# flanglet/kanzi

Measured on AMD Instinct MI355X. Metric: encode+decode MB/s, 4 MiB-block synthetic stream, BWT+RANK+ZRLT & ANS0 (level-5 core chain), bit-exact .knz, higher is better.
Workload: dtype u8; 1 GPU; configs[2]: BWT+RANK+ZRLT & ANS0, 2048 x 4194304 B blocks per GPU per step (64 distinct synthetic blocks per GPU, SURVEY 8d generator standing in for silesia.tar, tiled), blocks round-robin over ranks; block_size=4194304, parallelism=blocks%1, round_trip_ok=True

## Files before the change

kanzi_amd/csrc/kz_api.hip:

```cpp
#include <dirent.h>
#include "kz_pipe.h"
#include <stdlib.h>
#include <thread>
#include <sched.h>

extern "C" int32_t kz_abi_version(void) { return KZ_ABI_VERSION; }

extern "C" kz_ctx* kz_ctx_create(int32_t deviceId) {
  int ndev = 0;
  if (hipGetDeviceCount(&ndev) != hipSuccess || ndev <= 0) return nullptr;
  if (deviceId < 0 || deviceId >= ndev) return nullptr;
  if (hipSetDevice(deviceId) != hipSuccess) return nullptr;
  kz_ctx* ctx = new kz_ctx();
  ctx->device = deviceId;
  { int cus = 0; if (hipDeviceGetAttribute(&cus, hipDeviceAttributeMultiprocessorCount, deviceId) == hipSuccess && cus > 0) ctx->numCUs = cus; }
  if (hipStreamCreateWithFlags(&ctx->stream, hipStreamNonBlocking) != hipSuccess) { delete ctx; return nullptr; }
  if (hipHostMalloc((void**)&ctx->hpin, 1 << 20, hipHostMallocDefault) != hipSuccess) { hipStreamDestroy(ctx->stream); delete ctx; return nullptr; }
  ctx->hpinInts = (1 << 20) / 4;
  kz_switches_read(ctx->sw);
  {
    const int hw = (int)std::thread::hardware_concurrency();
    ctx->blockingWaits = ctx->sw.blockingWaits >= 0 ? ctx->sw.blockingWaits : ((hw > 0 && kz_usable_cpus() < hw) ? 1 : 0);
  }
  return ctx;
}
void kz_switches_read(kz_switches& s) {
  s = kz_switches();
  auto num = [](const char* name, int unset) { const char* e = getenv(name); return e ? atoi(e) : unset; };
  auto flag = [](const char* name) { return getenv(name) != nullptr ? 1 : 0; };
  auto digit = [](const char* name, int lo, int hi, int unset) { const char* e = getenv(name); return (e && e[0] >= '0' + lo && e[0] <= '0' + hi) ? e[0] - '0' : unset; };
  { const char* e = getenv("KZ_BLOCKING_WAITS"); s.blockingWaits = e ? (atoi(e) ? 1 : 0) : -1; }
  s.textGpu = digit("KZ_TEXT_GPU", 0, 3, -1);
  s.textGpuMin = num("KZ_TEXT_GPU_MIN", 512);
  s.textFwdGpu = digit("KZ_TEXT_FWD_GPU", 0, 1, -1);
  s.textFwdGpuMin = num("KZ_TEXT_FWD_GPU_MIN", 256);
  s.text1FwdGpu = digit("KZ_TEXT1_FWD_GPU", 0, 1, -1);
  s.text1FwdGpuMin = num("KZ_TEXT1_FWD_GPU_MIN", 64);
  s.utfGpu = digit("KZ_UTF_GPU", 0, 0, 1);
  s.utfFwdGpu = digit("KZ_UTF_FWD_GPU", 0, 1, -1);
  s.textGpuTrace = flag("KZ_TEXT_GPU_TRACE");
  s.fuseMinBlocks = num("KZ_FUSE_MIN_BLOCKS", 32);
  s.overlapClasses = num("KZ_OVERLAP_CLASSES", 3);
  { const char* e = getenv("KZ_WIDE_QUEUES"); s.wideQueues = e ? (atoi(e) ? 1 : 0) : -1; }
  s.noSFirst = flag("KZ_NO_SFIRST");
  s.traceSched = flag("KZ_TRACE_SCHED");
  s.tracePipe = flag("KZ_TRACE_PIPE");
  s.hostChunk = num("KZ_HOST_CHUNK", 0);
  { const int v = num("KZ_HOST_CHUNK_DEC", 512); s.hostChunkDec = v < 8 ? 8 : v; }
  { const char* e = getenv("KZ_HOST_INV_STAGED"); s.hostInvStaged = e ? atoi(e) : -1; }
  s.streamChunk = num("KZ_STREAM_CHUNK", 0);
  s.streamSerial = flag("KZ_STREAM_SERIAL");
  s.readScatter = flag("KZ_READ_SCATTER");
  s.writeGather = flag("KZ_WRITE_GATHER");
  s.bwtTrie = num("KZ_BWT_TRIE", -1); s.bwtTrieWin = num("KZ_BWT_TRIEWIN", -1); s.bwtBuckets = num("KZ_BWT_BUCKETS", -1);
  s.bwtDmax = num("KZ_BWT_DMAX", -1); s.bwtRetire = num("KZ_BWT_RETIRE", -1); s.bwtLazyRank = num("KZ_BWT_LAZYRANK", -1);
  s.bwtTrace = flag("KZ_BWT_TRACE");
  s.bwtTestTrieOverflow = digit("KZ_BWT_TEST_TRIE_OVERFLOW", 0, 9, -1);
  s.cmTestRowBytes = num("KZ_CM_TEST_ROW_BYTES", 0);
  { const char* f = getenv("KZ_FPAQ_FORCE"); s.fpaqForce = f ? ((f[0] == 'w' || f[0] == 'W' || f[0] == '1') ? 1 : ((f[0] == 'l' || f[0] == 'L' || f[0] == '2') ? 2 : 0)) : 0; }
  s.sbrtForm = num("KZ_SBRT_FORM", -1);
}
extern "C" void kz_ctx_reload_switches(kz_ctx* ctx) {
  if (!ctx) return;
  kz_switches_read(ctx->sw);
  if (ctx->sw.blockingWaits >= 0) ctx->blockingWaits = ctx->sw.blockingWaits;
}
extern "C" void kz_ctx_destroy(kz_ctx* ctx) {
  if (!ctx) return;
  if (ctx->worker.joinable()) {
    { std::lock_guard<std::mutex> g(ctx->qmu); ctx->stopWorker = true; }
    ctx->qcv.notify_all();
    ctx->worker.join();
  }
  hipSetDevice(ctx->device);
  if (ctx->arena) hipFree(ctx->arena);
  for (int i = 0; i < 5; i++) { if (ctx->side[i]) hipStreamDestroy(ctx->side[i]); if (ctx->evJoin[i]) hipEventDestroy(ctx->evJoin[i]); }
  if (ctx->hpin) hipHostFree(ctx->hpin);
  for (int i = 0; i < 2; i++) {
    if (ctx->pinIn[i].p) hipHostFree(ctx->pinIn[i].p);
    if (ctx->pinOut[i].p) hipHostFree(ctx->pinOut[i].p);
    if (ctx->hsIn[i].p) hipHostFree(ctx->hsIn[i].p);
    if (ctx->hsOut[i].p) hipHostFree(ctx->hsOut[i].p);
    if (ctx->tfOut[i].p) hipHostFree(ctx->tfOut[i].p);
    if (ctx->hiAux[i].p) hipFree(ctx->hiAux[i].p);
    if (ctx->hiStream[i]) hipStreamDestroy(ctx->hiStream[i]);
    if (ctx->devIn[i].p) hipFree(ctx->devIn[i].p);
    if (ctx->devOut[i].p) hipFree(ctx->devOut[i].p);
  }
// ... 357 lines not shown
```

kanzi_amd/csrc/kz_bwt_fwd.h:

```cpp
#pragma once
#include "kz_device.h"
#include "kz_internal.h"
#include <utility>

#define BW_LIVE 0x80000000u

typedef unsigned long long u64;
typedef uint32_t u32;
typedef uint8_t u8;
typedef u64 __attribute__((aligned(1))) bw_u64_unaligned;

struct BwtArrays {
  u64* key[2]; u32* val[2];
  u32* rank; u32* sa;
  u32* tileHist;
  u32* digitBase;
  u32* bucketCnt;
  int32_t* d_w;
  int32_t* d_big;
  u32* tileA;
  u32* tileB;
  u32* tileLive;
  int32_t* d_n;
  int32_t* d_m;
// ... 135 lines not shown
      const u32 r1 = run + c0;
      if (c1) gdelta[j + 1] = V.bStart[j + 1] + atomicAdd(&V.bFill[j + 1], c1) - r1;
      tc2[j >> 1] = run | (r1 << 16);
      run = r1 + c1;
    }
    if (threadIdx.x == 0) scan[31] = total;
  }
  __syncthreads();
  const u32 total = scan[31];
#pragma unroll
  for (int r = 0; r < TILE_ / 1024; r++) {
    if (bp[r] != 0xFFFFFFFFu) {
      const u32 bk = bp[r] & 0xFFFFu;
      const u32 w = tc2[bk >> 1];
      const u32 slot = ((bk & 1u) ? (w >> 16) : (w & 0xFFFFu)) + (bp[r] >> 16);
      stage[slot] = el[r]; stageB[slot] = (uint16_t)bk;
    }
  }
  __syncthreads();
#pragma unroll
  for (int r = 0; r < TILE_ / 1024; r++) {
    const u32 slot = (u32)r * 1024 + threadIdx.x;
    if (slot < total) elem[gdelta[stageB[slot]] + slot] = stage[slot];
  }
}

struct BwtRun {
  kz_ctx* ctx; kz_batch* bt;
  BwtArrays A; TrieArrays TR;
  int B, maxN, T; int64_t NS;
  int bitsR, bitsG, nBuckets, Dmax;
  bool useBuckets, useTrie;
  bool noRetire, trieWinOff, lazyRank, trace; int forceOvfRound;
  u64 *kC, *kF; u32 *vC, *vF;
  void swap() { std::swap(kC, kF); std::swap(vC, vF); }
  int nAct;
  int32_t *h_act, *d_act;
  int mMax, wMax;
  int h; bool windowed;
};
static inline int gridFor(int n, int per) { int g = (n + per - 1) / per; return g < 1 ? 1 : g; }

bool tr_applies(int maxN);
size_t bwt_trie_scratch(int maxN);
bool bwt_trie_alloc(kz_ctx* ctx, int B, int maxN, TrieArrays& TR);
int bwt_trie_text_round(BwtRun& R);
int bwt_trie_key_round(BwtRun& R);
```

kanzi_amd/csrc/kz_bwt_fwd.hip:

```cpp
#include "kz_bwt_fwd.h"
#include <stdlib.h>
#include <algorithm>

#define RS_ITEMS 16
#define RS_TILE (KZ_WG * RS_ITEMS)
#define RSORT_TILE 16384
#define RSORT_ITEMS (RSORT_TILE / KZ_WG)

__device__ __forceinline__ u64 bw_text_key(const u8* __restrict__ s, int i, int n, int K) {
  u64 k = __builtin_bswap64(*(const bw_u64_unaligned*)(s + i)) >> (8 * (8 - K));
  const int rem = n - i;
  if (rem < K) k &= ~0ULL << (8 * (K - rem));
  return k;
}
struct TextSrc { const u8* src; int64_t stride; int K; };
__global__ void k_bwt_init(BwtArrays A, int B) {
  const int b = blockIdx.x * blockDim.x + threadIdx.x;
  if (b < B) { A.d_m[b] = A.d_n[b]; A.d_w[b] = 0; }
}

#define MSD_BINS 1024
template <int BINS, bool MSD, bool TEXT>
__device__ __forceinline__ void radix_hist_body(const u64* __restrict__ keyIn, const BwtArrays& A, int shift, TextSrc X) {
  const int b = bw_row_block(A, blockIdx.y);
// ... 12 lines not shown
    const int idx = base + r * KZ_WG + threadIdx.x;
    const bool valid = idx < m;
    const u32 d = valid ? (u32)(((TEXT ? bw_text_key(X.src + (int64_t)b * X.stride, idx, m, X.K) : key[idx]) >> shift) & (BINS - 1)) : 0;
    const uint64_t vm = kz_ballot(valid);
    const u32 d0 = (u32)__builtin_amdgcn_readfirstlane((int)d);
    if (vm != 0 && kz_ballot(valid && d == d0) == vm) { if (lane == (int)__builtin_ctzll(vm)) atomicAdd(&hist[d0], (u32)__popcll(vm)); }
    else if (valid) atomicAdd(&hist[d], 1u);
  }
  __syncthreads();
  u32* th = A.tileHist + (int64_t)b * A.HS + (int64_t)tile * BINS;
  for (int i = threadIdx.x; i < BINS; i += KZ_WG) th[i] = hist[i];
}
__global__ __launch_bounds__(KZ_WG) void k_radix_hist(const u64* __restrict__ keyIn, BwtArrays A, int shift) { radix_hist_body<256, false, false>(keyIn, A, shift, TextSrc{nullptr, 0, 0}); }
__global__ __launch_bounds__(KZ_WG) void k_radix_hist0(BwtArrays A, TextSrc X) { radix_hist_body<256, false, true>(nullptr, A, 0, X); }
__global__ __launch_bounds__(KZ_WG) void k_msd_hist(const u64* __restrict__ keyIn, BwtArrays A, int shift) { radix_hist_body<MSD_BINS, true, false>(keyIn, A, shift, TextSrc{nullptr, 0, 0}); }

__global__ __launch_bounds__(256) void k_radix_scan(BwtArrays A) {
  const int b = bw_row_block(A, blockIdx.x);
  const int m = A.d_m[b] - A.d_w[b];
  const int tiles = (m + RSORT_TILE - 1) / RSORT_TILE;
  __shared__ u32 lds[32];
  u32* h = A.tileHist + (int64_t)b * A.HS;
  u32 run = 0;
  for (int t = 0; t < tiles; t++) {
    u32 v = h[(int64_t)t * 256 + threadIdx.x];
    h[(int64_t)t * 256 + threadIdx.x] = run;
    run += v;
  }
  u32 total;
  u32 ex = kz_wg_excl_sum(run, lds, &total);
  A.digitBase[b * MSD_BINS + threadIdx.x] = ex;
}

__global__ __launch_bounds__(MSD_BINS) void k_msd_scan(BwtArrays A) {
  const int b = bw_row_block(A, blockIdx.x);
  const int m = A.d_m[b];
  const int tiles = (m + RSORT_TILE - 1) / RSORT_TILE;
  __shared__ u32 lds[32];
  u32* h = A.tileHist + (int64_t)b * A.HS;
  u32 run = 0;
  for (int t = 0; t < tiles; t++) {
    u32 v = h[(int64_t)t * MSD_BINS + threadIdx.x];
    h[(int64_t)t * MSD_BINS + threadIdx.x] = run;
    run += v;
  }
  const bool big = run > BK_CAP;
  u32 mSmall, mBig;
  const u32 exS = kz_wg_excl_sum(big ? 0u : run, lds, &mSmall);
  __syncthreads();
  const u32 exB = kz_wg_excl_sum(big ? run : 0u, lds, &mBig);
  A.digitBase[b * MSD_BINS + threadIdx.x] = big ? mSmall + exB : exS;
  A.bucketCnt[b * MSD_BINS + threadIdx.x] = big ? (run | BK_BIG) : run;
  if (threadIdx.x == 0) { A.d_w[b] = (int32_t)mSmall; A.d_big[b] = (int32_t)mBig; }
}

#define RSC_WAVES 16
#define RSC_ITEMS (RSORT_TILE / (64 * RSC_WAVES))
#define RSC_WG (64 * RSC_WAVES)
template <int BINS, int NBITS, bool MSD, typename CNT, bool TEXT>
__device__ __forceinline__ void radix_scatter_body(const u64* __restrict__ keyIn, const u32* __restrict__ valIn,
                                                   u64* __restrict__ keyOut, u32* __restrict__ valOut,
                                                   const BwtArrays& A, int shift, TextSrc X) {
  const int b = bw_row_block(A, blockIdx.y);
  const int w0 = MSD ? 0 : A.d_w[b];
  const int m = A.d_m[b] - w0;
  const int tile = blockIdx.x;
  if ((int64_t)tile * RSORT_TILE >= m) return;
  __shared__ CNT cnt[RSC_WAVES][BINS];
  __shared__ u32 gdelta[BINS];
  __shared__ u32 scan[32];
// ... 58 lines not shown
    if (idx < m) { const u32 slot = cnt[wave][dr[r] & 0xFFFF] + (dr[r] >> 16); dr[r] = slot; stage[slot] = k[r]; }
  }
  __syncthreads();
  u32 gp[RSC_ITEMS];
#pragma unroll
  for (int r = 0; r < RSC_ITEMS; r++) {
    const int slot = r * RSC_WG + threadIdx.x;
    if (slot < tcount) {
      const u64 kk = stage[slot];
      gp[r] = gdelta[(u32)((kk >> shift) & (BINS - 1))] + (u32)slot;
      keyOut[off + gp[r]] = kk;
    }
  }
  __syncthreads();
  u32* stageV = (u32*)stage;
#pragma unroll
  for (int r = 0; r < RSC_ITEMS; r++) {
    const int idx = base + r * 64 + lane;
    if (idx < m) stageV[dr[r]] = v[r];
  }
  __syncthreads();
#pragma unroll
  for (int r = 0; r < RSC_ITEMS; r++) {
    const int slot = r * RSC_WG + threadIdx.x;
    if (slot < tcount) valOut[off + gp[r]] = stageV[slot];
  }
}
__global__ __launch_bounds__(RSC_WG) void k_radix_scatter(const u64* __restrict__ keyIn, const u32* __restrict__ valIn,
                                                           u64* __restrict__ keyOut, u32* __restrict__ valOut,
                                                           BwtArrays A, int shift) { radix_scatter_body<256, 8, false, u32, false>(keyIn, valIn, keyOut, valOut, A, shift, TextSrc{nullptr, 0, 0}); }
__global__ __launch_bounds__(RSC_WG) void k_radix_scatter0(u64* __restrict__ keyOut, u32* __restrict__ valOut, BwtArrays A, TextSrc X) {
  radix_scatter_body<256, 8, false, u32, true>(nullptr, nullptr, keyOut, valOut, A, 0, X);
}
__global__ __launch_bounds__(RSC_WG) void k_msd_scatter(const u64* __restrict__ keyIn, const u32* __restrict__ valIn,
                                                         u64* __restrict__ keyOut, u32* __restrict__ valOut,
                                                         BwtArrays A, int shift) {
  const int b = bw_row_block(A, blockIdx.y);
  const int m = A.d_m[b];
  const int tile = blockIdx.x;
  if ((int64_t)tile * RSORT_TILE >= m) return;
  __shared__ u32 cnt[MSD_BINS];
  __shared__ u32 gdelta[MSD_BINS];
  __shared__ u32 scan[32];
  __shared__ u64 stage[RSORT_TILE];
  cnt[threadIdx.x] = 0;
  __syncthreads();
  const int64_t off = (int64_t)b * A.NS;
  const int lane = kz_lane();
  const int tbase = tile * RSORT_TILE;
  const int tcount = min(RSORT_TILE, m - tbase);
  const uint64_t lt = kz_lanemask_lt();
  u64 k[RSC_ITEMS]; u32 v[RSC_ITEMS]; u32 dr[RSC_ITEMS];
#pragma unroll
  for (int r = 0; r < RSC_ITEMS; r++) {
    const int idx = tbase + r * RSC_WG + threadIdx.x;
    const bool valid = idx < m;
    k[r] = valid ? keyIn[off + idx] : 0;
    v[r] = valid ? valIn[off + idx] : 0;
  }
#pragma unroll
  for (int r = 0; r < RSC_ITEMS; r++) {
    const int idx = tbase + r * RSC_WG + threadIdx.x;
    const bool valid = idx < m;
    const u32 d = (u32)(k[r] >> shift) & (MSD_BINS - 1);
    const uint64_t vm = kz_ballot(valid);
    const u32 d0 = (u32)__builtin_amdgcn_readfirstlane((int)d);
    u32 pos = 0;
    if (vm != 0 && kz_ballot(valid && d == d0) == vm) {
      u32 basePos = 0;
      if (lane == (int)__builtin_ctzll(vm)) basePos = atomicAdd(&cnt[d0], (u32)__popcll(vm));
      basePos = (u32)__shfl((int)basePos, (int)__builtin_ctzll(vm), 64);
      pos = basePos + (u32)__popcll(vm & lt);
    } else if (valid) pos = atomicAdd(&cnt[d], 1u);
    dr[r] = pos;
  }
  __syncthreads();
  {
    const u32 tot = cnt[threadIdx.x];
    u32 total;
    const u32 ts = kz_wg_excl_sum(tot, scan, &total);
    gdelta[threadIdx.x] = A.digitBase[b * MSD_BINS + threadIdx.x] + A.tileHist[(int64_t)b * A.HS + (int64_t)tile * MSD_BINS + threadIdx.x] - ts;
    cnt[threadIdx.x] = ts;
  }
  __syncthreads();
#pragma unroll
  for (int r = 0; r < RSC_ITEMS; r++) {
    const int idx = tbase + r * RSC_WG + threadIdx.x;
    if (idx < m) { const u32 slot = cnt[(u32)(k[r] >> shift) & (MSD_BINS - 1)] + dr[r]; dr[r] = slot; stage[slot] = k[r]; }
  }
  __syncthreads();
  u32 gp[RSC_ITEMS];
#pragma unroll
  for (int r = 0; r < RSC_ITEMS; r++) {
    const int slot = r * RSC_WG + threadIdx.x;
    if (slot < tcount) {
      const u64 kk = stage[slot];
      gp[r] = gdelta[(u32)(kk >> shift) & (MSD_BINS - 1)] + (u32)slot;
      keyOut[off + gp[r]] = kk;
    }
  }
  __syncthreads();
  u32* stageV = (u32*)stage;
#pragma unroll
  for (int r = 0; r < RSC_ITEMS; r++) {
    const int idx = tbase + r * RSC_WG + threadIdx.x;
    if (idx < m) stageV[dr[r]] = v[r];
  }
  __syncthreads();
#pragma unroll
  for (int r = 0; r < RSC_ITEMS; r++) {
    const int slot = r * RSC_WG + threadIdx.x;
    if (slot < tcount) valOut[off + gp[r]] = stageV[slot];
  }
}

__device__ __forceinline__ u32 bw_group(u64 k, int gshift) { return gshift >= 64 ? 0u : (u32)(k >> gshift); }

__device__ __forceinline__ void bw_row_flags(const u64* __restrict__ key, int base, int m, int gshift, int lane,
                                             u64 (&k)[RS_ITEMS], uint64_t (&hb)[RS_ITEMS], uint64_t (&sb)[RS_ITEMS]) {
  u64 prevRowLast = (base > 0 && base <= m) ? key[base - 1] : 0;
#pragma unroll
  for (int r = 0; r < RS_ITEMS; r++) {
    const int c = base + r * 64 + lane;
    k[r] = (c < m) ? key[c] : 0;
    u64 prev = __shfl_up(k[r], 1, 64);
    if (lane == 0) prev = prevRowLast;
    const bool valid = c < m;
    const bool head = valid && (c == 0 || k[r] != prev);
    const bool seg = head && (c == 0 || bw_group(k[r], gshift) != bw_group(prev, gshift));
    hb[r] = kz_ballot(head);
    sb[r] = kz_ballot(seg);
    prevRowLast = __shfl(k[r], 63, 64);
  }
}

__global__ __launch_bounds__(KZ_WG) void k_seg_reduce(const u64* __restrict__ keyS, BwtArrays A, int gshift) {
  const int b = bw_row_block(A, blockIdx.y);
  const int w0 = A.d_w[b];
  const int m = A.d_m[b] - w0;
  const int tile = blockIdx.x;
  if ((int64_t)tile * RS_TILE >= m) return;
  __shared__ u32 wS[4], wH[4];
  const u64* key = keyS + (int64_t)b * A.NS + w0;
  const int wave = threadIdx.x >> 6, lane = kz_lane();
  const int base = tile * RS_TILE + wave * (64 * RS_ITEMS);
  u64 k[RS_ITEMS]; uint64_t hb[RS_ITEMS], sb[RS_ITEMS];
// ... 389 lines not shown
    const int s = base + r * 64 + lane;
    rk[r] = (s < n) ? rank[s] : 0u;
    bal[r] = kz_ballot((rk[r] & BW_LIVE) != 0);
    if (lane == 0) rowCnt[wave * RS_ITEMS + r] = (u32)__popcll(bal[r]);
  }
  __syncthreads();
  if (threadIdx.x < 64) {
    const u32 v = rowCnt[threadIdx.x];
    const u32 inc = kz_wave_incl_sum(v);
    rowCnt[threadIdx.x] = inc - v;
    if (threadIdx.x == 63) {
      const u32 tot = inc;
      A.tileLive[(int64_t)b * A.T + tile] = tot;
      tileBase = tot ? (u32)atomicAdd(&A.d_m2[b], (int32_t)tot) : 0u;
    }
  }
  __syncthreads();
  const u32 tbase = tileBase;
  const uint64_t lt = kz_lanemask_lt();
  const u32 hcap = (u32)min(h, n);
#pragma unroll
  for (int r = 0; r < RS_ITEMS; r++) {
    if (rk[r] & BW_LIVE) {
      const int s = base + r * 64 + lane;
      const int64_t j = (int64_t)s + h;
      const u64 r2 = (j < n) ? (u64)(rank[j] & ~BW_LIVE) + (u64)hcap + 1ULL : (u64)(n - s);
      const u32 pos = tbase + rowCnt[wave * RS_ITEMS + r] + (u32)__popcll(bal[r] & lt);
      keyN[off + pos] = ((u64)(rk[r] & ~BW_LIVE) << bitsR) | r2;
      valN[off + pos] = (u32)s;
    }
  }
}


__global__ void k_bwt_emit(const u8* __restrict__ src, int64_t srcStride, u8* __restrict__ dst, int64_t dstStride,
                           BwtArrays A, int32_t* d_lenOut, int32_t* d_flag, int B) {
  const int lin = blockIdx.y * gridDim.x + blockIdx.x;
  const int sg = lin / (8 * (int)gridDim.x), r8 = lin % (8 * (int)gridDim.x);
  const int b = B < 0 ? (int)blockIdx.y : sg * 8 + (r8 & 7);
  const int chunk = B < 0 ? (int)blockIdx.x : r8 >> 3;
  if (B >= 0 && b >= B) return;
  const int n = A.d_n[b];
  const u8* s = src + (int64_t)b * srcStride;
  u8* d = dst + (int64_t)b * dstStride;
  const int64_t off = (int64_t)b * A.NS;
  if (n < 2) {
    if (chunk == 0 && threadIdx.x == 0) { d_flag[b] = 0; d_lenOut[b] = n; if (n == 1) d[0] = s[0]; }
    return;
  }
  int logBlockSize = kz_ilog2((u32)n);
  if ((n & (n - 1)) != 0) logBlockSize++;
  const int pIndexSize = (logBlockSize + 7) >> 3;
  const int chunks = (n < 256) ? 1 : 8;
  const int hdr = 1 + chunks * pIndexSize;
  const u32* rank = A.rank + off;
  const u32* sa = A.sa + off;
  const int p = (int)rank[0];
  if (chunk == 0 && threadIdx.x == 0) {
    const int logNbChunks = (chunks == 8) ? 3 : 0;
    d[0] = (u8)((logNbChunks << 2) | (pIndexSize - 1));
    const int st = n / chunks;
    const int step = (st * chunks != n) ? st + 1 : st;
    int idx = 1;
    for (int k = 0; k < chunks; k++) {
      const int pi = (int)rank[(int64_t)k * step];
      for (int shift = (pIndexSize - 1) << 3; shift >= 0; shift -= 8) d[idx++] = (u8)(pi >> shift);
// ... 38 lines not shown
  A.d_big = (int32_t*)take(B * 4);
  A.tileA = (u32*)take(T * B * 4);
  A.tileB = (u32*)take(T * B * 4);
  A.tileLive = (u32*)take(T * B * 4);
  A.d_m = (int32_t*)take(B * 4);
  A.d_m2 = (int32_t*)take(B * 4);
  R.d_act = (int32_t*)take(B * 4);
  return ok;
}

static const int BW_K0 = 7;
static const int BW_BUCKET_MIN = 4096;

static int bwt_plan(BwtRun& R, kz_ctx* ctx, kz_batch& bt, bool allowTrie) {
  R.ctx = ctx; R.bt = &bt; R.B = bt.B;
  for (int b = 0; b < bt.B; b++) if (bt.h_len[b] > R.maxN) R.maxN = bt.h_len[b];
  const int maxN = R.maxN;
  R.NS = (int64_t)kz_align((size_t)(maxN > 0 ? maxN : 1), RS_TILE);
  R.T = (int)(R.NS / RS_TILE);
  R.A.NS = R.NS; R.A.T = R.T; R.A.HS = (int64_t)((R.NS + RSORT_TILE - 1) / RSORT_TILE) * MSD_BINS;
  if (!bwt_alloc_arrays(R)) { snprintf(ctx->err, sizeof(ctx->err), "bwt_forward: arena overflow"); return -KZ_ERR_DEVICE; }
  R.useTrie = allowTrie && ctx->sw.bwtTrie != 0 && tr_applies(maxN) && bwt_trie_alloc(ctx, bt.B, maxN, R.TR);
  R.A.d_n = bt.d_len;
  R.bitsR = 1;
  while ((1LL << R.bitsR) < 2 * (int64_t)maxN + 2) R.bitsR++;
  R.bitsG = 1;
  while ((1LL << R.bitsG) < (int64_t)maxN) R.bitsG++;
  R.nBuckets = 1 << (R.bitsG > BK_BITS ? R.bitsG - BK_BITS : 0);
  R.useBuckets = (BK_BITS + R.bitsR + R.bitsG <= 64) && R.nBuckets <= MSD_BINS && ctx->sw.bwtBuckets != 0;
  R.Dmax = (ctx->sw.bwtDmax >= 6 && ctx->sw.bwtDmax <= TR_DMAX_LIMIT) ? ctx->sw.bwtDmax : 6;
  R.noRetire = ctx->sw.bwtRetire == 0;
  R.trieWinOff = ctx->sw.bwtTrieWin == 0;
  R.lazyRank = ctx->sw.bwtLazyRank != 0;
  R.trace = ctx->sw.bwtTrace != 0;
  R.forceOvfRound = ctx->sw.bwtTestTrieOverflow;
  R.kC = R.A.key[0]; R.kF = R.A.key[1]; R.vC = R.A.val[0]; R.vF = R.A.val[1];
  R.nAct = bt.B;
  R.h_act = ctx->hpin + bt.B + 16;
  R.mMax = maxN;
  return 0;
}

static int bwt_round_buckets(BwtRun& R, int round) {
  kz_ctx* ctx = R.ctx; BwtArrays& A = R.A;
  const int nAct = R.nAct, nBuckets = R.nBuckets;
  const int rt = gridFor(R.mMax, RSORT_TILE);
  const int sh = R.bitsR + BK_BITS;
  KZ_LAUNCH(ctx, KID_MSD_HIST, k_msd_hist, dim3(rt, nAct), dim3(KZ_WG), R.kC, A, sh);
  KZ_LAUNCH(ctx, KID_MSD_SCAN, k_msd_scan, dim3(nAct), dim3(MSD_BINS), A);
  KZ_HIP(hipMemcpyAsync(ctx->hpin, A.d_big, (size_t)R.B * 4, hipMemcpyDeviceToHost, ctx->stream));
  KZ_LAUNCH(ctx, KID_MSD_SCATTER, k_msd_scatter, dim3(rt, nAct), dim3(RSC_WG), R.kC, R.vC, R.kF, R.vF, A, sh);
  R.swap();
  KZ_LAUNCH(ctx, KID_BUCKET_COUNT_S, k_bucket_count_s, dim3(nBuckets, nAct), dim3(256), R.kC, R.vC, A, R.bitsR, R.bitsG, (u32)BK_GMAX);
  KZ_LAUNCH(ctx, KID_BUCKET_COUNT, k_bucket_count, dim3(nBuckets, nAct), dim3(1024), R.kC, R.vC, A, R.bitsR, R.bitsG, (u32)BK_GMAX);
  KZ_LAUNCH(ctx, KID_BUCKET_SORT, k_bucket_sort, dim3(nBuckets, nAct), dim3(1024), R.kC, R.vC, A, R.bitsR, R.bitsG);
  KZ_HIP(kz_stream_sync(ctx, ctx->stream));
  R.wMax = 0;
  long long tot = 0;
  for (int r = 0; r < nAct; r++) { const int w = ctx->hpin[A.act ? R.h_act[r] : r]; tot += w; if (w > R.wMax) R.wMax = w; }
  R.windowed = true;
  if (R.trace) fprintf(stderr, "[bwt] round %d: %lld suffixes in oversized buckets, max per block %d\n", round, tot, R.wMax);
  return 0;
}

static int bwt_round_lsd(BwtRun& R, int round) {
  kz_ctx* ctx = R.ctx; const BwtArrays& A = R.A;
  const int nAct = R.nAct;
  const int nbits = (round == 0) ? 8 * BW_K0 : R.bitsR + R.bitsG;
  const int passes = (nbits + 7) / 8;
  const int gshift = (round == 0) ? 64 : R.bitsR;
  const int tiles = gridFor(R.wMax, RS_TILE);
  const int rtiles = gridFor(R.wMax, RSORT_TILE);
  for (int p = 0; p < passes; p++) {
    if (round == 0 && p == 0) {
      const TextSrc X0 = {R.bt->buf[R.bt->cur], R.bt->stride, BW_K0};
      KZ_LAUNCH(ctx, KID_RADIX_HIST, k_radix_hist0, dim3(rtiles, nAct), dim3(KZ_WG), A, X0);
      KZ_LAUNCH(ctx, KID_RADIX_SCAN, k_radix_scan, dim3(nAct), dim3(256), A);
      KZ_LAUNCH(ctx, KID_RADIX_SCATTER, k_radix_scatter0, dim3(rtiles, nAct), dim3(RSC_WG), R.kF, R.vF, A, X0);
    } else {
      KZ_LAUNCH(ctx, KID_RADIX_HIST, k_radix_hist, dim3(rtiles, nAct), dim3(KZ_WG), R.kC, A, p * 8);
      KZ_LAUNCH(ctx, KID_RADIX_SCAN, k_radix_scan, dim3(nAct), dim3(256), A);
      KZ_LAUNCH(ctx, KID_RADIX_SCATTER, k_radix_scatter, dim3(rtiles, nAct), dim3(RSC_WG), R.kC, R.vC, R.kF, R.vF, A, p * 8);
    }
    R.swap();
  }
  KZ_LAUNCH(ctx, KID_SEG_REDUCE, k_seg_reduce, dim3(tiles, nAct), dim3(KZ_WG), R.kC, A, gshift);
  KZ_LAUNCH(ctx, KID_SEG_SCAN, k_seg_scan, dim3(nAct), dim3(64), A);
  KZ_LAUNCH(ctx, KID_SEG_APPLY, k_seg_apply, dim3(tiles, nAct), dim3(KZ_WG), R.kC, R.vC, A, gshift);
  return 0;
}

static int bwt_compact_and_read_back(BwtRun& R, int round, bool* trieOverflow) {
  kz_ctx* ctx = R.ctx; BwtArrays& A = R.A;
  const int B = R.B;
  hipStream_t st = ctx->stream;
  R.h = (round == 0) ? (R.useTrie ? 6 : BW_K0) : R.h * 2;
  KZ_HIP(hipMemsetAsync(A.d_m2, 0, (size_t)B * 4, st));
  KZ_LAUNCH(ctx, KID_LIVE_EMIT, k_live_emit, dim3(gridFor(R.maxN, RS_TILE), R.nAct), dim3(KZ_WG), R.kF, R.vF, A, R.h, R.bitsR, round == 0 ? 1 : 0,
            (round == 0 && R.useTrie && R.lazyRank) ? R.TR.meta : (const int32_t*)nullptr);
  R.swap();
  KZ_HIP(hipMemcpyAsync(ctx->hpin, A.d_m2, (size_t)B * 4, hipMemcpyDeviceToHost, st));
  ctx->hpin[B] = 0;
  if (R.useTrie) KZ_HIP(hipMemcpyAsync(ctx->hpin + B, R.TR.err, 4, hipMemcpyDeviceToHost, st));
  KZ_HIP(kz_stream_sync(ctx, st));
  R.mMax = 0;
  for (int b = 0; b < B; b++) if (ctx->hpin[b] > R.mMax) R.mMax = ctx->hpin[b];
  if (R.useTrie && (ctx->hpin[B] != 0 || round == R.forceOvfRound)) { *trieOverflow = true; return 0; }
  if (R.trace) {
    long long tot = 0, totN = 0; for (int b = 0; b < B; b++) { tot += ctx->hpin[b]; totN += R.bt->h_len[b]; }
    fprintf(stderr, "[bwt] round %d h=%d: live %lld of %lld (%.1f%%), max per block %d\n", round, R.h, tot, totN, 100.0 * tot / (totN ? totN : 1), R.mMax);
  }
  std::swap(A.d_m, A.d_m2);
  return 0;
}

static int bwt_retire(BwtRun& R) {
  kz_ctx* ctx = R.ctx;
  if (R.mMax <= 0 || R.noRetire) return 0;
  int cnt = 0;
  for (int b = 0; b < R.B; b++) if (ctx->hpin[b] > 0) R.h_act[cnt++] = b;
  if (cnt < R.B) {
    KZ_HIP(hipMemcpyAsync(R.d_act, R.h_act, (size_t)cnt * 4, hipMemcpyHostToDevice, ctx->stream));
    R.A.act = R.d_act;
    R.nAct = cnt;
  }
  return 0;
}

static int bwt_emit(BwtRun& R) {
  kz_ctx* ctx = R.ctx; kz_batch& bt = *R.bt;
  const int B = R.B;
  const int rows8 = (B + 7) / 8 * 8;
  const bool xcd = rows8 <= KZ_MAX_BATCH;
  KZ_LAUNCH(ctx, KID_BWT_EMIT, k_bwt_emit, dim3(gridFor(R.maxN, 256 * 8), xcd ? rows8 : B), dim3(256), bt.buf[bt.cur], bt.stride, bt.buf[bt.cur ^ 1], bt.stride,
            R.A, bt.d_len2, bt.d_flag, xcd ? B : -1);
  KZ_HIP(hipGetLastError());
  bt.cur ^= 1;
  std::swap(bt.d_len, bt.d_len2);
  return 0;
}

static int bwt_forward_run(kz_ctx* ctx, kz_batch& bt, bool allowTrie, bool* trieOverflow) {
  BwtRun R{};
  int rc = bwt_plan(R, ctx, bt, allowTrie);
  if (rc) return rc;
  KZ_LAUNCH(ctx, KID_BWT_INIT, k_bwt_init, dim3((R.B + 255) / 256), dim3(256), R.A, R.B);
// ... 32 lines not shown
```

kanzi_amd/csrc/kz_internal.h:

```cpp
#pragma once
#include <hip/hip_runtime.h>
#include <stdint.h>
#include <stdio.h>
#include <string.h>
#include <vector>
#include <condition_variable>
#include <deque>
#include <functional>
#include <map>
#include <set>
#include <mutex>
#include <thread>
#include "../../include/kanzi_hip.h"

#define KZ_KERNELS(X) \
  X(KID_ANS_ENC_CHUNK, "k_ans_enc_chunk") X(KID_ANS_ENC_SCAN, "k_ans_enc_scan") X(KID_ANS_ENC_CONCAT, "k_ans_enc_concat") X(KID_ANS_DEC_INDEX, "k_ans_dec_index") \
  X(KID_ANS_DEC_CHUNK, "k_ans_dec_chunk") X(KID_ANS_DEC_FIN, "k_ans_dec_fin") X(KID_MASK_LEN, "k_mask_len") X(KID_PASSTHROUGH, "k_passthrough") \
  X(KID_FRAME_PREPARE, "k_frame_prepare") X(KID_COPY_BYTES, "k_copy_bytes") X(KID_FRAME_DECIDE, "k_frame_decide") X(KID_FRAME_HEADER, "k_frame_header") \
  X(KID_FRAME_PARSE, "k_frame_parse") X(KID_COPY_PAYLOAD, "k_copy_payload") X(KID_BWT_INIT, "k_bwt_init") X(KID_RADIX_HIST, "k_radix_hist") \
  X(KID_RADIX_SCAN, "k_radix_scan") X(KID_RADIX_SCATTER, "k_radix_scatter") X(KID_SEG_REDUCE, "k_seg_reduce") X(KID_SEG_SCAN, "k_seg_scan") \
  X(KID_SEG_APPLY, "k_seg_apply") X(KID_LIVE_EMIT, "k_live_emit") X(KID_BWT_EMIT, "k_bwt_emit") X(KID_BWTI_PARSE, "k_bwti_parse") \
  X(KID_BWTI_HIST, "k_bwti_hist") X(KID_BWTI_SCAN, "k_bwti_scan") X(KID_BWTI_SCATTER, "k_bwti_scatter") X(KID_BWTI_WALK1, "k_bwti_walk1") \
  X(KID_BWTI_RESOLVE, "k_bwti_resolve") X(KID_BWTI_COPY, "k_bwti_copy") X(KID_BWTI_LITERAL, "k_bwti_literal") X(KID_BWTI_FIN, "k_bwti_fin") \
  X(KID_SBRT_LAST2, "k_sbrt_last2") X(KID_SBRT_SCAN, "k_sbrt_scan") X(KID_SBRT_REPLAY, "k_sbrt_replay") X(KID_COPY_LEN, "k_copy_len") \
// ... 25 lines not shown
  X(KID_KNZ_SCAN_COUNT, "k_knz_scan_count") X(KID_KNZ_SCAN_SUM, "k_knz_scan_sum") X(KID_KNZ_SCAN_WRITE, "k_knz_scan_write") X(KID_KNZ_SCAN_LINK, "k_knz_scan_link") \
  X(KID_KNZ_SCAN_RUN, "k_knz_scan_run") X(KID_KNZ_SCAN_MARK, "k_knz_scan_mark") X(KID_KNZ_SCAN_EMIT, "k_knz_scan_emit") X(KID_KNZ_CHECK_ROWS, "k_knz_check_rows") \
  X(KID_KNZ_SPLICE_MANY, "k_knz_splice_many")
#define KZ_KERNEL_ENUM(id, name) id,
#define KZ_KERNEL_NAME(id, name) name,
enum KzKernelId { KZ_KERNELS(KZ_KERNEL_ENUM) KID_COUNT };
#define KZ_KERNEL_NAMES { KZ_KERNELS(KZ_KERNEL_NAME) }
struct kz_switches {
  int blockingWaits = -1;
  int textGpu = -1;
  int textGpuMin = 512;
  int textFwdGpu = -1;
  int textFwdGpuMin = 256;
  int text1FwdGpu = -1;
  int text1FwdGpuMin = 64;
  int utfGpu = 1;
  int utfFwdGpu = -1;
  int textGpuTrace = 0;
  int fuseMinBlocks = 32;
  int overlapClasses = 3;
  int wideQueues = -1;
  int noSFirst = 0;
  int traceSched = 0;
  int tracePipe = 0;
  int hostChunk = 0;
  int hostChunkDec = 512;
  int hostInvStaged = -1;
  int streamChunk = 0;
  int streamSerial = 0;
  int readScatter = 0;
  int writeGather = 0;
  int bwtTrie = -1, bwtTrieWin = -1, bwtBuckets = -1, bwtDmax = -1, bwtRetire = -1;
  int bwtLazyRank = -1;
  int bwtTrace = 0;
  int bwtTestTrieOverflow = -1;
  int fpaqForce = 0;
  int cmTestRowBytes = 0;
  int sbrtForm = -1;
};
void kz_switches_read(kz_switches& s);

struct KzPending { hipEvent_t e0, e1; int id; };
struct kz_ctx {
  int device = 0;
  kz_switches sw;
  hipStream_t stream = nullptr;
  hipStream_t side[5] = {nullptr, nullptr, nullptr, nullptr, nullptr};
  hipEvent_t evJoin[5] = {nullptr, nullptr, nullptr, nullptr, nullptr};
  int wideQueues = -1;
  int wideNow = 0;
  uint8_t* arena = nullptr;
  size_t arenaCap = 0, arenaTop = 0;
  int32_t* hpin = nullptr;
  size_t hpinInts = 0;
  char err[512] = {0};
  float stageMs[KZ_MAX_STAGES] = {0};
  int64_t stageAlgBytes[KZ_MAX_STAGES] = {0};
  int nStages = 0;
  int checksum = 0;
  int skipBlocks = 0;
  int dataType = 0;
  int blockSize = 4 * 1024 * 1024;
  bool blockSizeSet = false;
  int entropy = KZ_E_NONE;
  int rltBlockSize = 0;
  int numCUs = 256;
// ... 204 lines not shown
```

Baseline: 5068 MB/s.

## Partition live BWT suffixes directly from ranks, skipping live-list emit and MSD histogram

Adds a live-partition mode, on by default, for the bucketed prefix-doubling BWT. A new k_live_hist kernel counts live suffixes and builds per-tile MSD histograms straight from the rank array. A new k_live_scatter kernel builds the doubled keys and scatters them into MSD buckets in the same pass. This removes the separate k_live_emit compaction and k_msd_hist passes when enough suffixes are live, at the cost of scanning every text tile instead of only the compacted live list. When few suffixes remain live, it falls back to emitting the live list.

```diff
diff --git a/kanzi_amd/csrc/kz_api.hip b/kanzi_amd/csrc/kz_api.hip
--- a/kanzi_amd/csrc/kz_api.hip
+++ b/kanzi_amd/csrc/kz_api.hip
@@ -54,6 +54,7 @@
   s.writeGather = flag("KZ_WRITE_GATHER");
   s.bwtTrie = num("KZ_BWT_TRIE", -1); s.bwtTrieWin = num("KZ_BWT_TRIEWIN", -1); s.bwtBuckets = num("KZ_BWT_BUCKETS", -1);
   s.bwtDmax = num("KZ_BWT_DMAX", -1); s.bwtRetire = num("KZ_BWT_RETIRE", -1); s.bwtLazyRank = num("KZ_BWT_LAZYRANK", -1);
+  s.bwtLivePart = num("KZ_BWT_LIVEPART", -1);
   s.bwtTrace = flag("KZ_BWT_TRACE");
   s.bwtTestTrieOverflow = digit("KZ_BWT_TEST_TRIE_OVERFLOW", 0, 9, -1);
   s.cmTestRowBytes = num("KZ_CM_TEST_ROW_BYTES", 0);
diff --git a/kanzi_amd/csrc/kz_bwt_fwd.h b/kanzi_amd/csrc/kz_bwt_fwd.h
--- a/kanzi_amd/csrc/kz_bwt_fwd.h
+++ b/kanzi_amd/csrc/kz_bwt_fwd.h
@@ -191,6 +191,7 @@
   int bitsR, bitsG, nBuckets, Dmax;
   bool useBuckets, useTrie;
   bool noRetire, trieWinOff, lazyRank, trace; int forceOvfRound;
+  int livePart; bool fromRanks;
   u64 *kC, *kF; u32 *vC, *vF;
   void swap() { std::swap(kC, kF); std::swap(vC, vF); }
   int nAct;
diff --git a/kanzi_amd/csrc/kz_bwt_fwd.hip b/kanzi_amd/csrc/kz_bwt_fwd.hip
--- a/kanzi_amd/csrc/kz_bwt_fwd.hip
+++ b/kanzi_amd/csrc/kz_bwt_fwd.hip
@@ -68,10 +68,10 @@
   A.digitBase[b * MSD_BINS + threadIdx.x] = ex;
 }
 
-__global__ __launch_bounds__(MSD_BINS) void k_msd_scan(BwtArrays A) {
+__global__ __launch_bounds__(MSD_BINS) void k_msd_scan(BwtArrays A, int byText) {
   const int b = bw_row_block(A, blockIdx.x);
   const int m = A.d_m[b];
-  const int tiles = (m + RSORT_TILE - 1) / RSORT_TILE;
+  const int tiles = ((byText ? (m > 0 ? A.d_n[b] : 0) : m) + RSORT_TILE - 1) / RSORT_TILE;
   __shared__ u32 lds[32];
   u32* h = A.tileHist + (int64_t)b * A.HS;
   u32 run = 0;
@@ -196,6 +196,61 @@
 __global__ __launch_bounds__(RSC_WG) void k_radix_scatter0(u64* __restrict__ keyOut, u32* __restrict__ valOut, BwtArrays A, TextSrc X) {
   radix_scatter_body<256, 8, false, u32, true>(nullptr, nullptr, keyOut, valOut, A, 0, X);
 }
+#define MSD_NONE 0xFFFFFFFFu
+__device__ __forceinline__ u32 msd_tile_place(u32* cnt, u32 d, bool valid, int lane, uint64_t lt) {
+  const uint64_t vm = kz_ballot(valid);
+  if (vm == 0) return MSD_NONE;
+  const int l0 = (int)__builtin_ctzll(vm);
+  const u32 d0 = (u32)__builtin_amdgcn_readlane((int)d, l0);
+  u32 pos = MSD_NONE;
+  if (kz_ballot(valid && d == d0) == vm) {
+    u32 basePos = 0;
+    if (lane == l0) basePos = atomicAdd(&cnt[d0], (u32)__popcll(vm));
+    basePos = (u32)__builtin_amdgcn_readlane((int)basePos, l0);
+    if (valid) pos = basePos + (u32)__popcll(vm & lt);
+  } else if (valid) pos = atomicAdd(&cnt[d], 1u);
+  return pos;
+}
+__device__ __forceinline__ void msd_tile_flush(const u64 (&k)[RSC_ITEMS], const u32 (&v)[RSC_ITEMS], u32 (&dr)[RSC_ITEMS], int shift,
+                                               u64* __restrict__ keyOut, u32* __restrict__ valOut, const BwtArrays& A, int b, int tile,
+                                               u32* cnt, u32* gdelta, u32* scan, u64* stage) {
+  __syncthreads();
+  u32 tcount;
+  {
+    const u32 tot = cnt[threadIdx.x];
+    const u32 ts = kz_wg_excl_sum(tot, scan, &tcount);
+    gdelta[threadIdx.x] = A.digitBase[b * MSD_BINS + threadIdx.x] + A.tileHist[(int64_t)b * A.HS + (int64_t)tile * MSD_BINS + threadIdx.x] - ts;
+    cnt[threadIdx.x] = ts;
+  }
+  __syncthreads();
+#pragma unroll
+  for (int r = 0; r < RSC_ITEMS; r++) {
+    if (dr[r] != MSD_NONE) { const u32 slot = cnt[(u32)(k[r] >> shift) & (MSD_BINS - 1)] + dr[r]; dr[r] = slot; stage[slot] = k[r]; }
+  }
+  __syncthreads();
+  u32 gp[RSC_ITEMS];
+#pragma unroll
+  for (int r = 0; r < RSC_ITEMS; r++) {
+    const u32 slot = (u32)r * RSC_WG + threadIdx.x;
+    if (slot < tcount) {
+      const u64 kk = stage[slot];
+      gp[r] = gdelta[(u32)(kk >> shift) & (MSD_BINS - 1)] + slot;
+      keyOut[gp[r]] = kk;
+    }
+  }
+  __syncthreads();
+  u32* stageV = (u32*)stage;
+#pragma unroll
+  for (int r = 0; r < RSC_ITEMS; r++) {
+    if (dr[r] != MSD_NONE) stageV[dr[r]] = v[r];
+  }
+  __syncthreads();
+#pragma unroll
+  for (int r = 0; r < RSC_ITEMS; r++) {
+    const u32 slot = (u32)r * RSC_WG + threadIdx.x;
+    if (slot < tcount) valOut[gp[r]] = stageV[slot];
+  }
+}
 __global__ __launch_bounds__(RSC_WG) void k_msd_scatter(const u64* __restrict__ keyIn, const u32* __restrict__ valIn,
                                                          u64* __restrict__ keyOut, u32* __restrict__ valOut,
                                                          BwtArrays A, int shift) {
@@ -212,7 +267,6 @@
   const int64_t off = (int64_t)b * A.NS;
   const int lane = kz_lane();
   const int tbase = tile * RSORT_TILE;
-  const int tcount = min(RSORT_TILE, m - tbase);
   const uint64_t lt = kz_lanemask_lt();
   u64 k[RSC_ITEMS]; u32 v[RSC_ITEMS]; u32 dr[RSC_ITEMS];
 #pragma unroll
@@ -225,57 +279,9 @@
 #pragma unroll
   for (int r = 0; r < RSC_ITEMS; r++) {
     const int idx = tbase + r * RSC_WG + threadIdx.x;
-    const bool valid = idx < m;
-    const u32 d = (u32)(k[r] >> shift) & (MSD_BINS - 1);
-    const uint64_t vm = kz_ballot(valid);
-    const u32 d0 = (u32)__builtin_amdgcn_readfirstlane((int)d);
-    u32 pos = 0;
-    if (vm != 0 && kz_ballot(valid && d == d0) == vm) {
-      u32 basePos = 0;
-      if (lane == (int)__builtin_ctzll(vm)) basePos = atomicAdd(&cnt[d0], (u32)__popcll(vm));
-      basePos = (u32)__shfl((int)basePos, (int)__builtin_ctzll(vm), 64);
-      pos = basePos + (u32)__popcll(vm & lt);
-    } else if (valid) pos = atomicAdd(&cnt[d], 1u);
-    dr[r] = pos;
-  }
-  __syncthreads();
-  {
-    const u32 tot = cnt[threadIdx.x];
-    u32 total;
-    const u32 ts = kz_wg_excl_sum(tot, scan, &total);
-    gdelta[threadIdx.x] = A.digitBase[b * MSD_BINS + threadIdx.x] + A.tileHist[(int64_t)b * A.HS + (int64_t)tile * MSD_BINS + threadIdx.x] - ts;
-    cnt[threadIdx.x] = ts;
-  }
-  __syncthreads();
-#pragma unroll
-  for (int r = 0; r < RSC_ITEMS; r++) {
-    const int idx = tbase + r * RSC_WG + threadIdx.x;
-    if (idx < m) { const u32 slot = cnt[(u32)(k[r] >> shift) & (MSD_BINS - 1)] + dr[r]; dr[r] = slot; stage[slot] = k[r]; }
-  }
-  __syncthreads();
-  u32 gp[RSC_ITEMS];
-#pragma unroll
-  for (int r = 0; r < RSC_ITEMS; r++) {
-    const int slot = r * RSC_WG + threadIdx.x;
-    if (slot < tcount) {
-      const u64 kk = stage[slot];
-      gp[r] = gdelta[(u32)(kk >> shift) & (MSD_BINS - 1)] + (u32)slot;
-      keyOut[off + gp[r]] = kk;
-    }
-  }
-  __syncthreads();
-  u32* stageV = (u32*)stage;
-#pragma unroll
-  for (int r = 0; r < RSC_ITEMS; r++) {
-    const int idx = tbase + r * RSC_WG + threadIdx.x;
-    if (idx < m) stageV[dr[r]] = v[r];
-  }
-  __syncthreads();
-#pragma unroll
-  for (int r = 0; r < RSC_ITEMS; r++) {
-    const int slot = r * RSC_WG + threadIdx.x;
-    if (slot < tcount) valOut[off + gp[r]] = stageV[slot];
-  }
+    dr[r] = msd_tile_place(cnt, (u32)(k[r] >> shift) & (MSD_BINS - 1), idx < m, lane, lt);
+  }
+  msd_tile_flush(k, v, dr, shift, keyOut + off, valOut + off, A, b, tile, cnt, gdelta, scan, stage);
 }
 
 __device__ __forceinline__ u32 bw_group(u64 k, int gshift) { return gshift >= 64 ? 0u : (u32)(k >> gshift); }
@@ -731,6 +737,110 @@
   }
 }
 
+static_assert(RSORT_TILE == 4 * RS_TILE && RSC_ITEMS == 16, "k_live_hist / k_live_scatter: four rows of a thread per sub-tile");
+__device__ __forceinline__ u32 live_subtiles(const BwtArrays& A, int b, int tile, int n, int first) {
+  u32 m = 0;
+#pragma unroll
+  for (int q = 0; q < 4; q++) {
+    const int sub = tile * 4 + q;
+    if ((int64_t)sub * RS_TILE < n && (first || A.tileLive[(int64_t)b * A.T + sub] != 0)) m |= 1u << q;
+  }
+  return m;
+}
+__global__ __launch_bounds__(RSC_WG) void k_live_hist(BwtArrays A, int first, const int32_t* __restrict__ lazyMeta) {
+  const int b = bw_row_block(A, blockIdx.y);
+  const int n = A.d_n[b];
+  const int tile = blockIdx.x;
+  if ((int64_t)tile * RSORT_TILE >= n) return;
+  u32* th = A.tileHist + (int64_t)b * A.HS + (int64_t)tile * MSD_BINS;
+  u32* tl = A.tileLive + (int64_t)b * A.T + tile * 4;
+  const bool inText = threadIdx.x < 4 && (int64_t)(tile * 4 + (int)threadIdx.x) * RS_TILE < n;
+  if (lazyMeta && lazyMeta[(int64_t)b * TR_META] == 256 && lazyMeta[(int64_t)b * TR_META + 18] == 0 && lazyMeta[(int64_t)b * TR_META + 20] == 0) {
+    th[threadIdx.x] = 0;
+    if (inText) tl[threadIdx.x] = 0;
+    return;
+  }
+  const u32 subs = live_subtiles(A, b, tile, n, first);
+  __shared__ u32 hist[MSD_BINS];
+  __shared__ u32 subLive[4];
+  hist[threadIdx.x] = 0;
+  if (threadIdx.x < 4) subLive[threadIdx.x] = 0;
+  __syncthreads();
+  if (subs) {
+    const u32* rank = A.rank + (int64_t)b * A.NS;
+    const int lane = kz_lane();
+    const int tbase = tile * RSORT_TILE;
+    const uint64_t lt = kz_lanemask_lt();
+    u32 rk[RSC_ITEMS];
+#pragma unroll
+    for (int r = 0; r < RSC_ITEMS; r++) {
+      const int s = tbase + r * RSC_WG + (int)threadIdx.x;
+      rk[r] = ((subs >> (r >> 2)) & 1u) && s < n ? rank[s] : 0u;
+    }
+    u32 c[4] = {0, 0, 0, 0};
+#pragma unroll
+    for (int r = 0; r < RSC_ITEMS; r++) {
+      const bool live = (rk[r] & BW_LIVE) != 0;
+      c[r >> 2] += (u32)__popcll(kz_ballot(live));
+      (void)msd_tile_place(hist, ((rk[r] & ~BW_LIVE) >> BK_BITS) & (MSD_BINS - 1), live, lane, lt);
+    }
+    if (lane == 0) {
+#pragma unroll
+      for (int q = 0; q < 4; q++) if (c[q]) atomicAdd(&subLive[q], c[q]);
+    }
+  }
+  __syncthreads();
+  th[threadIdx.x] = hist[threadIdx.x];
+  if (inText) tl[threadIdx.x] = subLive[threadIdx.x];
+  if (threadIdx.x == 0) {
+    const u32 tot = subLive[0] + subLive[1] + subLive[2] + subLive[3];
+    if (tot) atomicAdd(&A.d_m2[b], (int32_t)tot);
+  }
+}
+__global__ __launch_bounds__(RSC_WG) void k_live_scatter(u64* __restrict__ keyOut, u32* __restrict__ valOut, BwtArrays A, int h, int bitsR) {
+  const int b = bw_row_block(A, blockIdx.y);
+  const int n = A.d_n[b];
+  const int tile = blockIdx.x;
+  if ((int64_t)tile * RSORT_TILE >= n || A.d_m[b] <= 0) return;
+  const u32 subs = live_subtiles(A, b, tile, n, 0);
+  if (!subs) return;
+  __shared__ u32 cnt[MSD_BINS];
+  __shared__ u32 gdelta[MSD_BINS];
+  __shared__ u32 scan[32];
+  __shared__ u64 stage[RSORT_TILE];
+  cnt[threadIdx.x] = 0;
+  __syncthreads();
+  const int64_t off = (int64_t)b * A.NS;
+  const u32* rank = A.rank + off;
+  const int lane = kz_lane();
+  const int tbase = tile * RSORT_TILE;
+  const uint64_t lt = kz_lanemask_lt();
+  const u32 hcap = (u32)min(h, n);
+  u64 k[RSC_ITEMS]; u32 v[RSC_ITEMS]; u32 dr[RSC_ITEMS];
+#pragma unroll
+  for (int r = 0; r < RSC_ITEMS; r++) {
+    const int s = tbase + r * RSC_WG + (int)threadIdx.x;
+    v[r] = (u32)s;
+    dr[r] = ((subs >> (r >> 2)) & 1u) && s < n ? rank[s] : 0u;
+  }
+#pragma unroll
+  for (int r = 0; r < RSC_ITEMS; r++) {
+    k[r] = 0;
+    if (dr[r] & BW_LIVE) {
+      const int s = tbase + r * RSC_WG + (int)threadIdx.x;
+      const int64_t j = (int64_t)s + h;
+      const u64 r2 = (j < n) ? (u64)(rank[j] & ~BW_LIVE) + (u64)hcap + 1ULL : (u64)(n - s);
+      k[r] = ((u64)(dr[r] & ~BW_LIVE) << bitsR) | r2;
+    }
+  }
+#pragma unroll
+  for (int r = 0; r < RSC_ITEMS; r++) {
+    const bool live = (dr[r] & BW_LIVE) != 0;
+    dr[r] = msd_tile_place(cnt, ((dr[r] & ~BW_LIVE) >> BK_BITS) & (MSD_BINS - 1), live, lane, lt);
+  }
+  msd_tile_flush(k, v, dr, bitsR + BK_BITS, keyOut + off, valOut + off, A, b, tile, cnt, gdelta, scan, stage);
+}
+
 
 __global__ void k_bwt_emit(const u8* __restrict__ src, int64_t srcStride, u8* __restrict__ dst, int64_t dstStride,
                            BwtArrays A, int32_t* d_lenOut, int32_t* d_flag, int B) {
@@ -835,6 +945,7 @@
   R.noRetire = ctx->sw.bwtRetire == 0;
   R.trieWinOff = ctx->sw.bwtTrieWin == 0;
   R.lazyRank = ctx->sw.bwtLazyRank != 0;
+  R.livePart = ctx->sw.bwtLivePart < 0 ? 1 : ctx->sw.bwtLivePart;
   R.trace = ctx->sw.bwtTrace != 0;
   R.forceOvfRound = ctx->sw.bwtTestTrieOverflow;
   R.kC = R.A.key[0]; R.kF = R.A.key[1]; R.vC = R.A.val[0]; R.vF = R.A.val[1];
@@ -844,15 +955,24 @@
   return 0;
 }
 
+static int bwt_partition(BwtRun& R) {
+  kz_ctx* ctx = R.ctx; BwtArrays& A = R.A;
+  const int nAct = R.nAct;
+  const int rt = gridFor(R.fromRanks ? R.maxN : R.mMax, RSORT_TILE);
+  const int sh = R.bitsR + BK_BITS;
+  if (!R.fromRanks) KZ_LAUNCH(ctx, KID_MSD_HIST, k_msd_hist, dim3(rt, nAct), dim3(KZ_WG), R.kC, A, sh);
+  KZ_LAUNCH(ctx, KID_MSD_SCAN, k_msd_scan, dim3(nAct), dim3(MSD_BINS), A, R.fromRanks ? 1 : 0);
+  KZ_HIP(hipMemcpyAsync(ctx->hpin, A.d_big, (size_t)R.B * 4, hipMemcpyDeviceToHost, ctx->stream));
+  if (R.fromRanks) KZ_LAUNCH(ctx, KID_MSD_SCATTER, k_live_scatter, dim3(rt, nAct), dim3(RSC_WG), R.kF, R.vF, A, R.h, R.bitsR);
+  else KZ_LAUNCH(ctx, KID_MSD_SCATTER, k_msd_scatter, dim3(rt, nAct), dim3(RSC_WG), R.kC, R.vC, R.kF, R.vF, A, sh);
+  return 0;
+}
+
 static int bwt_round_buckets(BwtRun& R, int round) {
   kz_ctx* ctx = R.ctx; BwtArrays& A = R.A;
   const int nAct = R.nAct, nBuckets = R.nBuckets;
-  const int rt = gridFor(R.mMax, RSORT_TILE);
-  const int sh = R.bitsR + BK_BITS;
-  KZ_LAUNCH(ctx, KID_MSD_HIST, k_msd_hist, dim3(rt, nAct), dim3(KZ_WG), R.kC, A, sh);
-  KZ_LAUNCH(ctx, KID_MSD_SCAN, k_msd_scan, dim3(nAct), dim3(MSD_BINS), A);
-  KZ_HIP(hipMemcpyAsync(ctx->hpin, A.d_big, (size_t)R.B * 4, hipMemcpyDeviceToHost, ctx->stream));
-  KZ_LAUNCH(ctx, KID_MSD_SCATTER, k_msd_scatter, dim3(rt, nAct), dim3(RSC_WG), R.kC, R.vC, R.kF, R.vF, A, sh);
+  const int rc = bwt_partition(R);
+  if (rc) return rc;
   R.swap();
   KZ_LAUNCH(ctx, KID_BUCKET_COUNT_S, k_bucket_count_s, dim3(nBuckets, nAct), dim3(256), R.kC, R.vC, A, R.bitsR, R.bitsG, (u32)BK_GMAX);
   KZ_LAUNCH(ctx, KID_BUCKET_COUNT, k_bucket_count, dim3(nBuckets, nAct), dim3(1024), R.kC, R.vC, A, R.bitsR, R.bitsG, (u32)BK_GMAX);
@@ -893,15 +1013,34 @@
   return 0;
 }
 
+static int bwt_live_list(BwtRun& R, bool first) {
+  kz_ctx* ctx = R.ctx; BwtArrays& A = R.A;
+  KZ_HIP(hipMemsetAsync(A.d_m2, 0, (size_t)R.B * 4, ctx->stream));
+  KZ_LAUNCH(ctx, KID_LIVE_EMIT, k_live_emit, dim3(gridFor(R.maxN, RS_TILE), R.nAct), dim3(KZ_WG), R.kF, R.vF, A, R.h, R.bitsR, first ? 1 : 0,
+            (first && R.useTrie && R.lazyRank) ? R.TR.meta : (const int32_t*)nullptr);
+  R.swap();
+  return 0;
+}
+static int bwt_live_count(BwtRun& R, bool first) {
+  kz_ctx* ctx = R.ctx; BwtArrays& A = R.A;
+  KZ_HIP(hipMemsetAsync(A.d_m2, 0, (size_t)R.B * 4, ctx->stream));
+  KZ_LAUNCH(ctx, KID_MSD_HIST, k_live_hist, dim3(gridFor(R.maxN, RSORT_TILE), R.nAct), dim3(RSC_WG), A, first ? 1 : 0,
+            (first && R.useTrie && R.lazyRank) ? R.TR.meta : (const int32_t*)nullptr);
+  return 0;
+}
+static bool bwt_next_from_ranks(const BwtRun& R) {
+  if (!R.livePart || !R.useBuckets || R.mMax < BW_BUCKET_MIN) return false;
+  return R.livePart < 2 || (int64_t)R.mMax * R.livePart >= (int64_t)R.maxN;
+}
+
 static int bwt_compact_and_read_back(BwtRun& R, int round, bool* trieOverflow) {
   kz_ctx* ctx = R.ctx; BwtArrays& A = R.A;
   const int B = R.B;
   hipStream_t st = ctx->stream;
   R.h = (round == 0) ? (R.useTrie ? 6 : BW_K0) : R.h * 2;
-  KZ_HIP(hipMemsetAsync(A.d_m2, 0, (size_t)B * 4, st));
-  KZ_LAUNCH(ctx, KID_LIVE_EMIT, k_live_emit, dim3(gridFor(R.maxN, RS_TILE), R.nAct), dim3(KZ_WG), R.kF, R.vF, A, R.h, R.bitsR, round == 0 ? 1 : 0,
-            (round == 0 && R.useTrie && R.lazyRank) ? R.TR.meta : (const int32_t*)nullptr);
-  R.swap();
+  const bool count = R.livePart && R.useBuckets;
+  int rc = count ? bwt_live_count(R, round == 0) : bwt_live_list(R, round == 0);
+  if (rc) return rc;
   KZ_HIP(hipMemcpyAsync(ctx->hpin, A.d_m2, (size_t)B * 4, hipMemcpyDeviceToHost, st));
   ctx->hpin[B] = 0;
   if (R.useTrie) KZ_HIP(hipMemcpyAsync(ctx->hpin + B, R.TR.err, 4, hipMemcpyDeviceToHost, st));
@@ -914,7 +1053,9 @@
     fprintf(stderr, "[bwt] round %d h=%d: live %lld of %lld (%.1f%%), max per block %d\n", round, R.h, tot, totN, 100.0 * tot / (totN ? totN : 1), R.mMax);
   }
   std::swap(A.d_m, A.d_m2);
-  return 0;
+  R.fromRanks = bwt_next_from_ranks(R);
+  if (count && !R.fromRanks && R.mMax > 0) rc = bwt_live_list(R, false);
+  return rc;
 }
 
 static int bwt_retire(BwtRun& R) {
diff --git a/kanzi_amd/csrc/kz_internal.h b/kanzi_amd/csrc/kz_internal.h
--- a/kanzi_amd/csrc/kz_internal.h
+++ b/kanzi_amd/csrc/kz_internal.h
@@ -81,6 +81,7 @@
   int writeGather = 0;
   int bwtTrie = -1, bwtTrieWin = -1, bwtBuckets = -1, bwtDmax = -1, bwtRetire = -1;
   int bwtLazyRank = -1;
+  int bwtLivePart = -1;
   int bwtTrace = 0;
   int bwtTestTrieOverflow = -1;
   int fpaqForce = 0;
```

Result: faster. 5314 MB/s, median of 6 (+4.9%).
